# genometools/vstree

Hardware: AMD Instinct MI355X
Metric: queries/sec (100 bp queries, vmatch -mum -l 20 semantics, 3 Gbp ESA index resident in HBM) (higher is better)
Workload: dtype u8; 1 GPU; 3 Gbp synthetic DNA index, 10 M x 100 bp queries per GPU, -mum -l 20; index_bp=3000000000, queries_per_gpu=10000000, query_len=100, minlen=20, prefixlength=13, index_bytes_hbm=115012207262, reads_in_hbm=two bits per symbol, 32 bytes per read (vsa_pack_reads), parallelism=index replicated, queries sharded x1

## Files before the change

vstree_amd/csrc/esa_device.hpp:

```cpp
#pragma once

#include "vsa_internal.hpp"
#include <type_traits>

#define VSA_ISSPECIAL(c) ((c) >= (uint8_t) VSA_WILDCARD)

__device__ __forceinline__ uint64_t vsa_load8(const uint8_t *p)
{
  uint64_t v;
  __builtin_memcpy(&v, p, 8);
  return v;
}

struct vsa_u128
{
  uint64_t lo, hi;
};

__device__ __forceinline__ vsa_u128 vsa_load16(const void *p)
{
  vsa_u128 v;
  __builtin_memcpy(&v, p, 16);
  return v;
}
// ... 324 lines not shown
      uint32_t bits;
      __builtin_memcpy(&bits, ix.spec64 + (b >> 3), 4);
      bits >>= (uint32_t) (b & 7u);
      const uint64_t have = 25, want = blast - b + 1;
      const uint32_t mask = want >= have ? (1u << have) - 1u
                                         : (1u << want) - 1u;
      if ((bits & mask) != 0)
      {
        return false;
      }
      b += have;
    }
  }
  lcplen = l;
  return true;
}

struct PackedQuery
{
  uint64_t w[4];
  uint32_t valid;
};

__device__ __forceinline__ uint64_t vsa_pq_window(const PackedQuery &pq,
                                                  uint32_t at)
{
  const uint32_t i = at >> 5, sh = 2u * (at & 31u);
  const uint64_t a = i == 0 ? pq.w[0]
                            : (i == 1 ? pq.w[1]
                                      : (i == 2 ? pq.w[2]
                                                : (i == 3 ? pq.w[3] : 0))),
                 b = i == 0 ? pq.w[1]
                            : (i == 1 ? pq.w[2] : (i == 2 ? pq.w[3] : 0));
  return sh != 0 ? (a << sh) | (b >> (64 - sh)) : a;
}

template <int BLK>
__device__ __forceinline__ void vsa_pq_stage(const DevQueries &qs, uint64_t q0,
                                             uint32_t m, uint32_t *lds,
                                             PackedQuery &pq)
{
  const uint64_t nhere = q0 < qs.nq ? (qs.nq - q0 < (uint64_t) BLK
                                           ? qs.nq - q0
                                           : (uint64_t) BLK)
                                    : 0;
  const uint32_t bytes = (uint32_t) nhere * m;
  const uint8_t *src = qs.symbols + q0 * m;
  for (uint32_t i = threadIdx.x; 16 * i < bytes; i += BLK)
  {
    const vsa_u128 v = vsa_load16(src + 16 * (uint64_t) i);
    uint4 *dst = reinterpret_cast<uint4 *>(lds) + i;
    *dst = make_uint4((uint32_t) v.lo, (uint32_t) (v.lo >> 32),
                      (uint32_t) v.hi, (uint32_t) (v.hi >> 32));
  }
  __syncthreads();
  pq.w[0] = pq.w[1] = pq.w[2] = pq.w[3] = 0;
  pq.valid = 0;
  if (threadIdx.x < nhere)
  {
    const uint32_t *row = lds + threadIdx.x * (m >> 2);
    uint32_t firstbad = m;
#pragma unroll
    for (uint32_t j = 0; j < 32; j++)
    {
      if (4 * j < m)
      {
        const uint32_t x = row[j];
        const uint32_t bad = x & 0xFCFCFCFCu;
        if (bad != 0 && firstbad == m)
        {
          firstbad = 4 * j + ((uint32_t) __builtin_ctz(bad) >> 3);
        }
        pq.w[j >> 3] |= (uint64_t) (vsa_pack4top(x) >> 24)
                        << (56 - 8 * (j & 7));
      }
    }
    pq.valid = firstbad;
  }
}

__device__ __forceinline__ void vsa_pq_from_row(const DevQueries &qs,
                                                uint64_t q, uint32_t m,
                                                PackedQuery &pq, QSrc &src)
{
  const uint32_t W = qs.roww;
  const uint64_t *row = qs.rows + q * W;
  const vsa_u128 a = vsa_load16(row), b = vsa_load16(row + 2);
  const uint64_t last = W == 1 ? a.lo : (W == 2 ? a.hi : (W == 3 ? b.lo : b.hi));
  pq.w[0] = a.lo;
  pq.w[1] = W > 1 ? a.hi : 0;
  pq.w[2] = W > 2 ? b.lo : 0;
  pq.w[3] = W > 3 ? b.hi : 0;
  if (W == 1)
  {
    pq.w[0] &= ~0xFFull;
  } else if (W == 2)
  {
    pq.w[1] &= ~0xFFull;
  } else if (W == 3)
  {
    pq.w[2] &= ~0xFFull;
  } else
  {
    pq.w[3] &= ~0xFFull;
  }
  pq.valid = m;
  src.row = row;
  src.bytes = nullptr;
  src.pos = 0;
  src.m = (int32_t) m;
  if ((last & 0xFFu) != 0 && qs.nside > 0)
  {
    const uint64_t k = (a.lo >> 8) < qs.nside ? (a.lo >> 8) : qs.nside - 1;
    const uint8_t *sym = qs.side + k * (uint64_t) m;
    uint32_t firstbad = m;
    src.bytes = sym;
#pragma unroll
    for (int wi = 0; wi < 4; wi++)
    {
      uint64_t acc = 0;
      for (uint32_t k = 0; k < 32; k++)
      {
        const uint32_t j = 32u * (uint32_t) wi + k;
        if (j < m)
        {
          const uint8_t c = sym[j];
          if (c > 3 && firstbad == m)
          {
            firstbad = j;
          }
          acc |= (uint64_t) (c & 3u) << (62 - 2 * k);
        }
      }
      pq.w[wi] = acc;
    }
    pq.valid = firstbad;
  }
}

struct RowQuery
{
  const uint64_t *row;
  uint32_t valid;
};

__device__ __forceinline__ uint64_t vsa_pq_window(const RowQuery &rq,
                                                  uint32_t at)
{
  const uint32_t i = at >> 5, sh = 2u * (at & 31u);
  const vsa_u128 w = vsa_load16(rq.row + i);
  return sh != 0 ? (w.lo << sh) | (w.hi >> (64 - sh)) : w.lo;
}

__device__ __forceinline__ bool vsa_row_of(const DevQueries &qs, uint64_t q,
                                           uint32_t m, RowQuery &rq,
                                           QSrc &src)
{
  const uint32_t W = qs.roww;
  rq.row = qs.rows + q * W;
  rq.valid = m;
  src.row = rq.row;
  src.bytes = nullptr;
  src.pos = 0;
  src.m = (int32_t) m;
  const bool flagged = (rq.row[W - 1] & 0xFFu) != 0 && qs.nside > 0;
  if (flagged)
  {
    const uint64_t k0 = rq.row[0] >> 8,
                   k = k0 < qs.nside ? k0 : qs.nside - 1;
    src.bytes = qs.side + k * (uint64_t) m;
  }
  return flagged;
}

__device__ __forceinline__ uint8_t vsa_pq_symbol(const PackedQuery &pq,
                                                 uint32_t i)
{
  return (uint8_t) (vsa_pq_window(pq, i) >> 62);
}

template <int CHUNKS, typename IDX, typename QT>
__device__ __forceinline__ bool
vsa_extend_packed_pq(const DevIndex<IDX> &ix, uint64_t sufstart,
                     const QT &pq, uint32_t pqoff,
                     uint32_t querylen, uint32_t &lcplen)
{
  const uint32_t from = lcplen,
                 left = pq.valid > pqoff ? pq.valid - pqoff : 0;
  uint32_t l = lcplen, qeff = querylen < left ? querylen : left;
  bool open = true;

  if ((uint64_t) qeff > ix.n - sufstart)
  {
    qeff = (uint32_t) (ix.n - sufstart);
  }
  while (open && l < qeff)
  {
    uint64_t A[CHUNKS][2];
#pragma unroll
    for (int c = 0; c < CHUNKS; c++)
    {
      const uint32_t lc = l + 60u * (uint32_t) c;
      A[c][0] = A[c][1] = 0;
      if (c == 0 || lc < qeff)
      {
        const uint64_t pos = sufstart + lc;
        const uint32_t sh = 2u * (uint32_t) (pos & 3u);
        const vsa_u128 t = vsa_load16(ix.tis2 + (pos >> 2));
        const uint64_t t0 = __builtin_bswap64(t.lo),
                       t1 = __builtin_bswap64(t.hi);
        A[c][0] = sh != 0 ? (t0 << sh) | (t1 >> (64 - sh)) : t0;
        A[c][1] = t1 << sh;
      }
    }
#pragma unroll
    for (int c = 0; c < CHUNKS; c++)
    {
      if (open && l < qeff)
      {
        const uint64_t x0 = A[c][0] ^ vsa_pq_window(pq, pqoff + l),
                       x1 = (A[c][1] ^ vsa_pq_window(pq, pqoff + l + 32)) &
                            ~0xFFull;
        uint32_t same = 60;
        if (x0 != 0)
        {
          same = (uint32_t) __builtin_clzll(x0) >> 1;
        } else if (x1 != 0)
        {
          same = 32 + ((uint32_t) __builtin_clzll(x1) >> 1);
        }
        l += same;
        open = same == 60;
      }
    }
  }
  if (l > qeff)
  {
    l = qeff;
  }
  if (sufstart + l + 64 >= ix.firstspecial)
  {
    uint64_t b = (sufstart + from) >> 6;
    const uint64_t blast = (sufstart + l) >> 6;
    while (b <= blast)
    {
      uint32_t bits;
      __builtin_memcpy(&bits, ix.spec64 + (b >> 3), 4);
      bits >>= (uint32_t) (b & 7u);
      const uint64_t have = 25, want = blast - b + 1;
      const uint32_t mask = want >= have ? (1u << have) - 1u
                                         : (1u << want) - 1u;
      if ((bits & mask) != 0)
      {
        return false;
      }
      b += have;
    }
  }
  lcplen = l;
  return true;
}

template <typename IDX, bool KEYED>
__device__ __forceinline__ uint64_t vsa_sufstart(const DevIndex<IDX> &ix,
                                                 uint64_t i)
{
  return (KEYED && sizeof(IDX) == 4) ? (ix.esa8[i] & 0xFFFFFFFFull)
                                     : (uint64_t) ix.suf[i];
}

template <typename IDX>
__device__ __forceinline__ uint64_t vsa_entrystart(const DevIndex<IDX> &ix,
                                                   uint64_t entry, uint64_t w)
{
  if constexpr (sizeof(IDX) == 4)
  {
    return entry & 0xFFFFFFFFull;
  } else
  {
    return (uint64_t) ix.suf[w];
  }
}

#define VSA_WIDE_LEFTBITS 40
template <typename IDX>
__device__ __forceinline__ void vsa_slotbounds(uint64_t b, uint64_t &left,
                                               uint32_t &cnt)
{
  if constexpr (sizeof(IDX) == 4)
  {
    const uint32_t dl = (uint32_t) b, dm = (uint32_t) (b >> 32);
    left = dl;
    cnt = (dm > dl) ? dm - dl : 0;
  } else
  {
    left = b & ((1ull << VSA_WIDE_LEFTBITS) - 1);
    cnt = (uint32_t) (b >> VSA_WIDE_LEFTBITS);
  }
}

template <typename IDX, bool KEYED>
__device__ __forceinline__ uint32_t vsa_lcpbyte(const DevIndex<IDX> &ix,
                                                uint64_t i)
{
  return KEYED ? (uint32_t) (ix.esa8[i] >> 32) & 0xFFu : (uint32_t) ix.lcp[i];
}
// ... 89 lines not shown
    {
      return mid;
    }
  }
  return l;
}

template <typename IDX>
__device__ __forceinline__ uint64_t vsa_largelcp(const DevIndex<IDX> &ix,
                                                 uint64_t i)
{
  uint64_t lo = 0, hi = ix.nllv;

  while (lo < hi)
  {
    const uint64_t mid = lo + ((hi - lo) >> 1);
    const uint64_t k = (uint64_t) ix.llv[2 * mid];
    if (i < k)
    {
      hi = mid;
    } else if (i > k)
    {
      lo = mid + 1;
    } else
    {
      return (uint64_t) ix.llv[2 * mid + 1];
    }
  }
  return 255;
}

template <typename IDX>
__device__ __forceinline__ uint64_t vsa_evallcp(const DevIndex<IDX> &ix,
                                                uint64_t i)
{
  const uint64_t v = ix.lcp[i];
  return (v < 255) ? v : vsa_largelcp(ix, i);
}

template <typename IDX, typename QP = const uint8_t *>
__device__ __forceinline__ bool vsa_qgram2code(const DevIndex<IDX> &ix,
                                               QP qgram, uint64_t &code)
{
  uint64_t c = 0;
  bool ok = true;

  if (ix.numofchars == 4)
  {
    for (uint32_t i = 0; i < ix.pl; i++)
    {
      const uint8_t a = vsa_qsym(qgram, i);
      ok = ok && !VSA_ISSPECIAL(a);
      c = (c << 2) | (a & 3);
    }
  } else
  {
    for (uint32_t i = 0; i < ix.pl; i++)
    {
      const uint8_t a = vsa_qsym(qgram, i);
      ok = ok && !VSA_ISSPECIAL(a);
      c = c * ix.numofchars + a;
    }
  }
  code = c;
  return ok;
}

template <typename IDX, typename QP = const uint8_t *>
__device__ __forceinline__ bool vsa_bucket(const DevIndex<IDX> &ix, QP qgram,
                                           uint64_t &vleft, uint64_t &vright)
{
  uint64_t code;

  if (!vsa_qgram2code(ix, qgram, code))
  {
    return false;
  }
  vleft = (uint64_t) ix.bck[2 * code];
  vright = (uint64_t) ix.bck[2 * code + 1];
  if (vright <= vleft)
  {
    return false;
  }
  vright--;
  return true;
}

template <typename IDX, typename QP = const uint8_t *>
__device__ __forceinline__ bool
vsa_locate_reference(const DevIndex<IDX> &ix, QP query, uint32_t querylen,
                     uint32_t &maxlcp, uint64_t &witness)
{
  uint64_t vleft, vright;

  if (!vsa_bucket(ix, query, vleft, vright))
  {
    return false;
  }
  vsa_findmaxprefixlen(ix, vleft, vright, ix.pl, query, querylen, maxlcp,
                       witness);
  return true;
}


__device__ __forceinline__ uint64_t vsa_pack8(uint64_t w)
{
  uint64_t x = __builtin_bswap64(w) & 0x0303030303030303ull;
  x = (x | (x >> 6)) & 0x000F000F000F000Full;
  x = (x | (x >> 12)) & 0x000000FF000000FFull;
  x = (x | (x >> 24)) & 0xFFFFull;
  return x;
}

__device__ __forceinline__ uint32_t vsa_keylcp(uint32_t a, uint32_t b,
                                               uint32_t nsyms)
{
  const uint32_t x = (a ^ b) & ((1u << (2 * nsyms)) - 1u);
  if (x == 0)
  {
    return nsyms;
  }
  const uint32_t h = 31u - (uint32_t) __builtin_clz(x);
  return (2 * nsyms - 1 - h) >> 1;
}

enum
{
  VSA_LOC_NONE = 0,
  VSA_LOC_FOUND = 1,
  VSA_LOC_SLOW = 2
};

__device__ __forceinline__ uint64_t vsa_ld_entry(const uint64_t *p)
{
  return *p;
}

struct DeepHit
{
  uint64_t ew;
  uint32_t lcpnext;
  uint8_t leftsym;
  bool notleftmax;
};

struct DeepFront
{
  uint64_t left;
  uint64_t first;
  uint32_t cnt, qkey, limit;
  int state;
};

template <bool PQ = false, typename IDX = uint32_t, typename QT = PackedQuery,
          typename QP = const uint8_t *>
__device__ __forceinline__ void
vsa_deep_front(const DevIndex<IDX> &ix, bool active, QP query,
               uint32_t querylen, DeepFront &f,
               const QT *pq = nullptr, uint32_t pqoff = 0)
{
  const uint32_t D = ix.D;
  f.state = VSA_LOC_NONE;
  f.left = 0;
  f.cnt = f.qkey = f.limit = 0;
  f.first = 0;
  if (active)
  {
    uint32_t valid = 32;
    uint64_t S = 0;
    if (PQ)
    {
      const uint32_t left = pq->valid > pqoff ? pq->valid - pqoff : 0;
      valid = left < 32 ? left : 32;
      S = vsa_pq_window(*pq, pqoff);
    } else
    {
      const vsa_u128 qlo = vsa_load16(query), qhi = vsa_load16(query + 16u);
      const uint64_t w0 = qlo.lo, w1 = qlo.hi, w2 = qhi.lo, w3 = qhi.hi;
      const uint64_t notdna = 0xFCFCFCFCFCFCFCFCull;
      const uint64_t s0 = w0 & notdna, s1 = w1 & notdna, s2 = w2 & notdna,
                     s3 = w3 & notdna;
      if ((s0 | s1 | s2 | s3) != 0)
      {
        if (s0 != 0)
        {
          valid = (uint32_t) __builtin_ctzll(s0) >> 3;
        } else if (s1 != 0)
        {
          valid = 8 + ((uint32_t) __builtin_ctzll(s1) >> 3);
        } else if (s2 != 0)
        {
          valid = 16 + ((uint32_t) __builtin_ctzll(s2) >> 3);
        } else
        {
          valid = 24 + ((uint32_t) __builtin_ctzll(s3) >> 3);
        }
      }
      S = ((uint64_t) vsa_pack16(w0, w1) << 32) | vsa_pack16(w2, w3);
    }
    if (valid > querylen)
    {
      valid = querylen;
    }
    if (valid < ix.pl)
    {
      f.state = VSA_LOC_NONE;
    } else if (valid < D)
    {
      f.state = VSA_LOC_SLOW;
    } else
    {
      const uint64_t code = S >> (64 - 2 * D);
      f.qkey = (uint32_t) (S >> (64 - 2 * D - 2 * VSA_KEYSYMS)) & VSA_KEYMASK;
      f.limit = valid - D;
      if (f.limit > VSA_KEYSYMS)
      {
        f.limit = VSA_KEYSYMS;
      }
      const vsa_u128 sl = vsa_load16(ix.slot16 + 2 * code);
      f.first = sl.hi;
      vsa_slotbounds<IDX>(sl.lo, f.left, f.cnt);
      f.state = (f.cnt > 0) ? VSA_LOC_FOUND : VSA_LOC_NONE;
    }
  }
}

template <int AHEAD, bool PQ, typename IDX, typename QT,
          typename QP = const uint8_t *>
__device__ __forceinline__ void
vsa_extend_tie(const DevIndex<IDX> &ix, uint64_t sstart, QP query,
               uint32_t querylen, uint32_t &maxlcp, const QT *pq,
               uint32_t pqoff)
{
  uint32_t lcplen = maxlcp;
  bool done = false;
  if (ix.tis2 != nullptr)
  {
    if constexpr (PQ)
    {
      done = vsa_extend_packed_pq<(AHEAD > 1 ? 2 : 1)>(ix, sstart, *pq, pqoff,
                                                       querylen, lcplen);
    } else
    {
      done = vsa_extend_packed<(AHEAD > 1 ? 2 : 1)>(ix, sstart, query,
                                                    querylen, lcplen);
    }
  }
  if (!done)
  {
    lcplen = maxlcp;
    (void) vsa_compare32<IDX, AHEAD>(ix, sstart, query, querylen, lcplen);
  }
  maxlcp = lcplen;
}

template <int AHEAD = 1, bool PQ = false, typename IDX = uint32_t,
          typename QT = PackedQuery, typename QP = const uint8_t *>
__device__ __forceinline__ int
vsa_locate_deep_from(const DevIndex<IDX> &ix, const DeepFront &f, QP query,
                     uint32_t querylen, uint32_t &maxlcp,
                     uint64_t &w, DeepHit &hit, uint32_t needleft = 0xFFFFFFFFu,
                     uint32_t qleft = 0x100u, const QT *pq = nullptr,
                     uint32_t pqoff = 0)
{
  const uint32_t D = ix.D;
  int state = f.state;
  const typename std::conditional<sizeof(IDX) == 4, uint32_t, uint64_t>::type
      dl = (typename std::conditional<sizeof(IDX) == 4, uint32_t,
                                      uint64_t>::type) f.left;
  const uint32_t cnt = f.cnt, qkey = f.qkey, limit = f.limit;
  const uint64_t first = f.first;

  const bool searching = state == VSA_LOC_FOUND;
  const uint32_t qk = qkey >> (2 * (VSA_KEYSYMS - limit));

  const bool small = searching && cnt <= 4;
  const uint32_t ksh = 2 * (VSA_KEYSYMS - limit);
  uint64_t e[5] = {0, 0, 0, 0, 0};
  if (small && cnt == 1)
  {
    e[0] = first;
  } else if (small)
  {
    const uint64_t *p = ix.esa8 + (uint64_t) dl + 1;
    const vsa_u128 e12 = vsa_load16(p);
    e[0] = first;
    e[1] = e12.lo;
    e[2] = e12.hi;
    if (cnt > 2)
    {
      const vsa_u128 e34 = vsa_load16(p + 2);
      e[3] = e34.lo;
      e[4] = e34.hi;
    }
  }
  uint32_t lo = 0;
  bool flagged = false;
  bool anylong = false, allnotleft = true;
  const uint32_t enough = needleft < D + limit ? needleft : D + limit;
  if (small)
  {
#pragma unroll
    for (uint32_t i = 0; i < 4; i++)
    {
      if (i < cnt)
      {
        flagged = flagged || (e[i] & VSA_KEYFLAG) != 0;
        const uint32_t tk =
            ((uint32_t) (e[i] >> VSA_KEYSHIFT) & VSA_KEYMASK) >> ksh;
        lo += (tk < qk) ? 1u : 0u;
        if (qleft < 0x100u)
        {
          const bool islong = D + vsa_keylcp(tk, qk, limit) >= enough;
          const bool sameleft =
              (e[i] & VSA_LEFTSPECIAL) == 0 &&
              (uint32_t) ((e[i] >> VSA_LEFTSHIFT) & 3u) == qleft;
          anylong = anylong || islong;
          allnotleft = allnotleft && (!islong || sameleft);
        }
      }
    }
  }
  uint32_t hi = (searching && !small) ? cnt : 0;
  uint32_t maxcnt = hi;
  if (__ballot(hi != 0) != 0)
  {
#pragma unroll
    for (int d = 32; d >= 1; d >>= 1)
    {
      const uint32_t o = __shfl_xor(maxcnt, d, 64);
      maxcnt = o > maxcnt ? o : maxcnt;
    }
  }
  for (uint32_t span = maxcnt; span > 0; span >>= 1)
  {
    if (lo < hi)
    {
      const uint32_t mid = (lo + hi) >> 1;
      const uint64_t em = vsa_ld_entry(ix.esa8 + (uint64_t) dl + mid);
      flagged = flagged || (em & VSA_KEYFLAG) != 0;
      const uint32_t tk =
          ((uint32_t) (em >> VSA_KEYSHIFT) & VSA_KEYMASK) >> ksh;
      if (tk < qk)
      {
        lo = mid + 1;
      } else
      {
        hi = mid;
      }
    }
  }
  uint64_t epred = 0, esucc = 0, enext = 0;
  bool haspred = false, hassucc = false, hasnext = false;
  if (searching)
  {
    haspred = lo > 0;
    hassucc = lo < cnt;
    hasnext = lo + 1 < cnt;
    if (small)
    {
      epred = lo == 1 ? e[0] : (lo == 2 ? e[1] : (lo == 3 ? e[2] : e[3]));
      esucc = lo == 0 ? e[0]
                      : (lo == 1 ? e[1]
                                 : (lo == 2 ? e[2] : (lo == 3 ? e[3] : e[4])));
      enext = lo == 0 ? e[1] : (lo == 1 ? e[2] : (lo == 2 ? e[3] : e[4]));
    } else
    {
      const uint64_t base = (uint64_t) dl + lo;
      if (base > 0)
      {
        epred = vsa_ld_entry(ix.esa8 + base - 1);
      }
      if (base <= ix.n)
      {
        esucc = vsa_ld_entry(ix.esa8 + base);
      }
      if (base + 1 <= ix.n)
// ... 229 lines not shown
```

vstree_amd/csrc/mum_walk.inc:

```
template <typename IDX, bool DEEP, bool PQ, typename QP>
__device__ __forceinline__ void
vsa_walk_step(const DevIndex<IDX> &ix, const DevQueries &qs, bool &active,
              QP read, const RowQuery *rq, uint32_t qlen, uint32_t first,
              uint32_t &off, uint64_t q, const uint64_t *__restrict__ base,
              uint32_t perquery, uint32_t searchlength,
              vsa_match *__restrict__ out, uint64_t *__restrict__ outkey,
              uint64_t shardcap, uint32_t shard,
              unsigned long long *__restrict__ cursors, uint32_t packbits,
              uint32_t valbits, uint32_t &locates)
{
  uint32_t c = 0, maxlcp = 0;
  uint64_t witness = 0;
  uint8_t leftchar = (uint8_t) VSA_SEPARATOR;
  const uint32_t remaining = qlen - off;
  const QP qptr = read + off;
  bool have = false, fast = false;
  DeepHit hit;
  int st = VSA_LOC_SLOW;
  locates += active ? 1u : 0u;
  if (active && off > 0)
  {
    if constexpr (PQ)
    {
      leftchar = (uint8_t) (vsa_pq_window(*rq, off - 1) >> 62);
    } else
    {
      leftchar = vsa_qsym(read, off - 1);
    }
  }
  if constexpr (DEEP)
  {
    const uint32_t qleft = off > 0 ? (uint32_t) leftchar : 0x100u;
    if constexpr (PQ)
    {
      st = vsa_locate_deep<1, true>(ix, active, qptr, remaining, maxlcp,
                                    witness, hit, searchlength, qleft, rq,
                                    off);
    } else
    {
      st = vsa_locate_deep(ix, active, qptr, remaining, maxlcp, witness,
                           hit, searchlength, qleft);
    }
  }
  if (st == VSA_LOC_SLOW)
  {
    have = active &&
           vsa_locate_reference(ix, qptr, remaining, maxlcp, witness);
  } else
  {
    have = st == VSA_LOC_FOUND;
    fast = have && maxlcp < 255;
  }
  const bool cutshort = st != VSA_LOC_SLOW && hit.notleftmax;
  if (have && maxlcp >= searchlength && !cutshort)
  {
    if (fast)
    {
      const uint32_t lcpw = (uint32_t) (hit.ew >> 32) & 0xFFu;
      const bool unique = (witness == 0 || lcpw < maxlcp) &&
                          (witness + 1 > ix.n - 1 || hit.lcpnext < maxlcp);
      c = (unique && (VSA_ISSPECIAL(leftchar) || leftchar != hit.leftsym))
              ? 1u
              : 0u;
    } else
    {
      c = (vsa_mum_candidate<IDX, DEEP>(ix, maxlcp, witness) &&
           vsa_leftmaximal(ix, vsa_sufstart<IDX, DEEP>(ix, witness),
                           leftchar))
              ? 1u
              : 0u;
    }
  }
  const uint64_t inshard = vsa_wave_reserve01(
      cursors + (uint64_t) shard * VSA_CURSOR_STRIDE, c != 0);
  if (c != 0 && inshard < shardcap)
  {
    const uint64_t dbstart = fast ? vsa_entrystart(ix, hit.ew, witness)
                                  : vsa_sufstart<IDX, DEEP>(ix, witness);
    const uint64_t t0 = (base != nullptr) ? base[q] : q * perquery;
    vsa_write_candidate(qs, out, outkey,
                        (uint64_t) shard * shardcap + inshard, q, off,
                        t0 + off, dbstart, maxlcp, packbits, valbits);
  }
  if (active)
  {
    uint32_t bound;
    if (st == VSA_LOC_SLOW)
    {
      bound = have ? maxlcp : ix.pl - 1;
    } else
    {
      bound = have ? maxlcp : ix.D - 1;
    }
    const uint32_t reach = off + bound;
    uint32_t next = off - 1;
    bool left = off > first;
    if (!cutshort && reach + 1 < off + searchlength)
    {
      left = left && reach >= searchlength;
      next = reach - searchlength;
    }
    active = left && next >= first;
    off = next;
  }
}

template <typename IDX, bool DEEP, bool PQ, typename QP>
__device__ __forceinline__ uint32_t
vsa_walk_chunk(const DevIndex<IDX> &ix, const DevQueries &qs, bool active,
               QP read, const RowQuery *rq, uint32_t qlen, uint32_t first,
               uint32_t off, uint64_t q, const uint64_t *__restrict__ base,
               uint32_t perquery, uint32_t searchlength,
               vsa_match *__restrict__ out, uint64_t *__restrict__ outkey,
               uint64_t shardcap, uint32_t shard,
               unsigned long long *__restrict__ cursors, uint32_t packbits,
               uint32_t valbits)
{
  uint32_t locates = 0;
  while (__any(active))
  {
    vsa_walk_step<IDX, DEEP, PQ>(ix, qs, active, read, rq, qlen, first, off, q,
                                 base, perquery, searchlength, out, outkey,
                                 shardcap, shard, cursors, packbits, valbits,
                                 locates);
  }
  return locates;
}
```

vstree_amd/csrc/mum_workplan.inc:

```



#define VSA_PLAN_RANGES 4
#define VSA_PLAN_ROUNDS 6
#define VSA_PLAN_UNKNOWN 0xFFFFFFFFu

#ifndef VSA_PLAN_WAVES
#define VSA_PLAN_WAVES 1
#endif
#ifndef VSA_FIRST_WAVES
#define VSA_FIRST_WAVES 1
#endif
struct PlanRanges
{
  uint32_t r[VSA_PLAN_RANGES];
};

__device__ __forceinline__ void plan_add(PlanRanges &pr, uint32_t &nr,
                                         uint32_t first, uint32_t last)
{
  if (first > last)
  {
    return;
  }
// ... 389 lines not shown
      rel[0] = 0;
    }
    __syncthreads();
    for (uint32_t d = 1; d < BLK; d <<= 1)
    {
      const uint64_t v = (tid + 1 > d) ? lanesum[tid + 1 - d] : 0;
      __syncthreads();
      lanesum[tid + 1] += v;
      __syncthreads();
    }
#pragma unroll
    for (int k = 0; k < RPT; k++)
    {
      rel[tid * RPT + k + 1] = (uint32_t) lanesum[tid] + mine[k];
    }
    __syncthreads();
  }
  const uint32_t total = rel[RPB];
  if (tid == 0)
  {
    if constexpr (MUM)
    {
      blocksum[vsa_bid()].offsets = lanesum[BLK] >> 32;
    } else
    {
      blocksum[vsa_bid()] = PlannedWork{total, total};
    }
  }
  const uint32_t shard = vsa_bid() & shardmask;
  uint32_t locates = 0;
  for (uint32_t i0 = 0; i0 < total; i0 += BLK)
  {
    const uint32_t i = i0 + tid;
    bool active = i < total;
    uint32_t off = 0, first = 0, qlen = qs.uniformlen;
    uint64_t q = 0, t0 = 0;
    const uint8_t *qstart = qs.symbols;
    if (active)
    {
      uint32_t lo = 0, hi = RPB;
      while (hi - lo > 1)
      {
        const uint32_t mid = (lo + hi) >> 1;
        if (rel[mid] <= i)
        {
          lo = mid;
        } else
        {
          hi = mid;
        }
      }
      uint32_t r = i - rel[lo];
#pragma unroll
      for (int k = 0; k < VSA_PLAN_RANGES; k++)
      {
        const uint32_t rf = pr[lo].r[k] & 0xFFFFu, len = pr[lo].r[k] >> 16,
                       nchunks = (len + chunk - 1) >> cshift;
        if (r < nchunks)
        {
          const uint32_t at = r << cshift,
                         n = len - at < chunk ? len - at : chunk;
          first = rf + at;
          off = first + n - 1;
          r = 0xFFFFFFFFu;
        } else if (r != 0xFFFFFFFFu)
        {
          r -= nchunks;
        }
      }
      q = q0 + lo;
      if constexpr (!MUM)
      {
        t0 = (base != nullptr) ? base[q] : q * perquery;
      }
      if constexpr (MUM && !ROWS)
      {
        if (qs.dense)
        {
          qstart = qs.symbols + q * qs.uniformlen;
        } else
        {
          qstart = qs.symbols + qs.start[q];
          qlen = (uint32_t) qs.length[q];
        }
      }
    }
    if constexpr (!MUM)
    {
      vsa_query_item<IDX, false, DEEP>(ix, qs, active, q, off, t0 + off,
                                       searchlength, out, outkey, shardcap,
                                       shard, cursors, 0, 0);
      continue;
    }
    if constexpr (DEEP && ROWS)
    {
      RowQuery rq;
      QSrc src;
      bool flagged = false;
      rq.row = qs.rows;
      rq.valid = 0;
      src.row = qs.rows;
      src.bytes = nullptr;
      src.pos = src.m = 0;
      if (active)
      {
        flagged = vsa_row_of(qs, q, qs.uniformlen, rq, src);
      }
      locates += vsa_walk_chunk<IDX, true, true>(
          ix, qs, active && !flagged, src, &rq, qlen, first, off, q, base,
          perquery, searchlength, out, outkey, shardcap, shard, cursors,
          packbits, valbits);
      if (__any(active && flagged))
      {
        locates += vsa_walk_chunk<IDX, true, false>(
            ix, qs, active && flagged, src, nullptr, qlen, first, off, q, base,
            perquery, searchlength, out, outkey, shardcap, shard, cursors,
            packbits, valbits);
      }
    } else
    {
      locates += vsa_walk_chunk<IDX, DEEP, false>(
          ix, qs, active, qstart, nullptr, qlen, first, off, q, base, perquery,
          searchlength, out, outkey, shardcap, shard, cursors, packbits,
          valbits);
    }
  }
  if constexpr (MUM)
  {
#pragma unroll
    for (int d = 32; d >= 1; d >>= 1)
    {
      locates += __shfl_xor(locates, d, 64);
    }
    if ((tid & 63u) == 0)
    {
      wavelocates[tid >> 6] = locates;
    }
    __syncthreads();
    if (tid == 0)
    {
      uint32_t s = 0;
#pragma unroll
      for (int w = 0; w < BLK / 64; w++)
      {
        s += wavelocates[w];
      }
      blocksum[vsa_bid()].locates = s;
    }
  }
}

struct WalkTile
{
  PlanRanges pr[64];
  uint32_t q[64];
  uint32_t pre[65];
};
#define VSA_WALK_ASIDE 128
struct WalkAside
{
  uint32_t q[VSA_WALK_ASIDE], r[VSA_WALK_ASIDE];
};

__device__ __forceinline__ void vsa_wave_lds_fence()
{
  __builtin_amdgcn_fence(__ATOMIC_RELEASE, "wavefront");
  __builtin_amdgcn_wave_barrier();
  __builtin_amdgcn_fence(__ATOMIC_ACQUIRE, "wavefront");
}

__device__ __forceinline__ uint32_t vsa_rank_in(uint64_t mask)
{
  return __builtin_amdgcn_mbcnt_hi(
      (uint32_t) (mask >> 32), __builtin_amdgcn_mbcnt_lo((uint32_t) mask, 0u));
}

__device__ __forceinline__ void vsa_plan_chunk(const PlanRanges &p, uint32_t r,
                                               uint32_t cshift,
                                               uint32_t &first, uint32_t &off)
{
  const uint32_t chunk = 1u << cshift;
#pragma unroll
  for (int k = 0; k < VSA_PLAN_RANGES; k++)
  {
    const uint32_t rf = p.r[k] & 0xFFFFu, len = p.r[k] >> 16,
                   nchunks = (len + chunk - 1) >> cshift;
    if (r < nchunks)
    {
      const uint32_t at = r << cshift, n = len - at < chunk ? len - at : chunk;
      first = rf + at;
      off = first + n - 1;
      r = 0xFFFFFFFFu;
    } else if (r != 0xFFFFFFFFu)
    {
      r -= nchunks;
    }
  }
}

template <typename IDX, bool DEEP = true, bool ROWS = false>
__global__ void __launch_bounds__(256, VSA_WALK_WAVES)
k_mum_walk_tiles(const DevIndex<IDX> ix, const DevQueries qs,
                 const uint64_t *__restrict__ base, uint32_t perquery,
                 const PlanRanges *__restrict__ plan,
                 const uint32_t *__restrict__ plancount,
                 const uint32_t *__restrict__ list,
                 const uint64_t *__restrict__ nlistword,
                 unsigned long long *__restrict__ tilecounter,
                 uint32_t searchlength, vsa_match *__restrict__ out,
                 uint64_t *__restrict__ outkey, uint64_t shardcap,
                 uint32_t shardmask, unsigned long long *__restrict__ cursors,
                 uint32_t packbits, uint32_t valbits,
                 PlannedWork *__restrict__ blocksum, uint32_t chunkshift)
{
  __shared__ WalkTile tiles[4];
  __shared__ WalkAside asides[ROWS ? 4 : 1];
  const uint32_t lane = threadIdx.x & 63u, wave = threadIdx.x >> 6;
  WalkTile &tile = tiles[wave];
  WalkAside &aside = asides[ROWS ? wave : 0];
  const uint64_t nlist = *nlistword & 0xFFFFFFFFull;
  const uint32_t shard = vsa_bid() & shardmask;
  uint32_t head = 0, tail = 0, naside = 0;
  bool exhausted = false;
  bool active = false;
  uint32_t off = 0, first = 0, q = 0, qlen = qs.uniformlen;
  uint32_t locates = 0, offsets = 0;
  const uint8_t *qstart = qs.symbols;
  for (;;)
  {
    uint64_t freemask = __ballot(!active);
    while (freemask != 0 && !(ROWS && naside >= 64))
    {
      if (head == tail)
      {
        if (exhausted)
        {
          break;
        }
        unsigned long long mine = 0;
        if (lane == 0)
        {
          mine = atomicAdd(tilecounter, 1ull);
        }
        const uint64_t t0 =
            ((uint64_t) __builtin_amdgcn_readfirstlane((uint32_t) (mine >> 32))
             << 32) |
            __builtin_amdgcn_readfirstlane((uint32_t) mine);
        if (t0 * 64 >= nlist)
        {
          exhausted = true;
          break;
        }
        const uint64_t t = t0 * 64 + lane;
        uint32_t tq = 0, nch = 0;
        PlanRanges p;
#pragma unroll
        for (int g = 0; g < VSA_PLAN_RANGES; g++)
        {
          p.r[g] = 0;
        }
        if (t < nlist)
        {
          tq = list[t];
          const uint32_t c = plancount[tq];
          p = plan[tq];
          offsets += c;
          if (c > 0)
          {
#pragma unroll
            for (int g = 0; g < VSA_PLAN_RANGES; g++)
            {
              nch += ((p.r[g] >> 16) + (1u << chunkshift) - 1) >> chunkshift;
            }
          }
        }
        const uint32_t incl = vsa_wave_inclusive_sum(nch);
        vsa_wave_lds_fence();
        tile.q[lane] = tq;
        tile.pr[lane] = p;
        tile.pre[lane + 1] = incl;
        if (lane == 0)
        {
          tile.pre[0] = 0;
        }
        vsa_wave_lds_fence();
        head = 0;
        tail = __builtin_amdgcn_readlane(incl, 63);
        continue;
      }
      const uint32_t nfree = (uint32_t) __popcll(freemask),
                     take = nfree < tail - head ? nfree : tail - head,
                     rank = vsa_rank_in(freemask);
      const bool took = !active && rank < take;
      bool flagged = false;
      if (took)
      {
        const uint32_t i = head + rank;
        uint32_t lo = 0;
#pragma unroll
        for (uint32_t d = 32; d >= 1; d >>= 1)
        {
          if (tile.pre[lo + d] <= i)
          {
            lo += d;
          }
        }
        q = tile.q[lo];
        vsa_plan_chunk(tile.pr[lo], i - tile.pre[lo], chunkshift, first, off);
        if constexpr (ROWS)
        {
          RowQuery rq;
          QSrc src;
          flagged = vsa_row_of(qs, q, qs.uniformlen, rq, src);
        } else
        {
          if (qs.dense)
          {
            qstart = qs.symbols + (uint64_t) q * qs.uniformlen;
          } else
          {
            qstart = qs.symbols + qs.start[q];
            qlen = (uint32_t) qs.length[q];
          }
        }
        active = !flagged;
      }
      head += take;
      if constexpr (ROWS)
      {
        const uint64_t fmask = __ballot(flagged);
        if (flagged)
        {
          const uint32_t at = naside + vsa_rank_in(fmask);
          aside.q[at] = q;
          aside.r[at] = first | (off << 16);
        }
        naside += (uint32_t) __popcll(fmask);
      }
      freemask = __ballot(!active);
    }
    if (!__any(active))
    {
      if constexpr (ROWS)
      {
        if (naside > 0)
        {
          vsa_wave_lds_fence();
          for (uint32_t a0 = 0; a0 < naside; a0 += 64)
          {
            const bool mine = a0 + lane < naside;
            uint32_t aq = 0, afirst = 0, aoff = 0;
            RowQuery arq;
            QSrc src;
            arq.row = qs.rows;
            arq.valid = 0;
            src.row = qs.rows;
            src.bytes = nullptr;
            src.pos = src.m = 0;
            if (mine)
            {
              aq = aside.q[a0 + lane];
              afirst = aside.r[a0 + lane] & 0xFFFFu;
              aoff = aside.r[a0 + lane] >> 16;
              (void) vsa_row_of(qs, aq, qs.uniformlen, arq, src);
            }
            locates += vsa_walk_chunk<IDX, true, false>(
                ix, qs, mine, src, nullptr, qlen, afirst, aoff, aq, base,
                perquery, searchlength, out, outkey, shardcap, shard, cursors,
                packbits, valbits);
          }
          vsa_wave_lds_fence();
          naside = 0;
          q = first = off = 0;
          continue;
        }
      }
      break;
    }
    if constexpr (DEEP && ROWS)
    {
      RowQuery rq;
      QSrc src;
      rq.row = qs.rows + (uint64_t) q * qs.roww;
      rq.valid = qlen;
      src.row = rq.row;
      src.bytes = nullptr;
      src.pos = 0;
      src.m = (int32_t) qlen;
      vsa_walk_step<IDX, true, true>(ix, qs, active, src, &rq, qlen, first,
                                     off, q, base, perquery, searchlength, out,
                                     outkey, shardcap, shard, cursors, packbits,
                                     valbits, locates);
    } else
    {
      vsa_walk_step<IDX, DEEP, false>(ix, qs, active, qstart, nullptr, qlen,
                                      first, off, q, base, perquery,
                                      searchlength, out, outkey, shardcap,
                                      shard, cursors, packbits, valbits,
                                      locates);
    }
  }
  uint64_t sum = locates | ((uint64_t) offsets << 32);
#pragma unroll
  for (int d = 32; d >= 1; d >>= 1)
  {
    sum += vsa_shfl64(sum, (int) lane ^ d);
  }
  if (lane == 0)
  {
    blocksum[vsa_bid() * 4 + wave] =
        PlannedWork{sum & 0xFFFFFFFFull, sum >> 32};
  }
}

template <typename IDX, bool DEEP, bool PQ = false, bool ROWS = false,
          bool WINDOWS = false>
__global__ void __launch_bounds__(VSA_BLOCK, VSA_FIRST_WAVES)
k_mum_first(const DevIndex<IDX> ix, const DevQueries qs, uint32_t perquery,
            uint32_t searchlength, uint32_t *__restrict__ count,
            uint32_t *__restrict__ firste, uint32_t *__restrict__ fmlen,
            uint64_t *__restrict__ fmdb,
            uint64_t *__restrict__ blockcount = nullptr)
{
  extern __shared__ uint32_t stagedqueries[];
  __shared__ uint32_t wantwaves[VSA_BLOCK / 64], candwaves[VSA_BLOCK / 64];
  const uint64_t q = vsa_bid() * VSA_BLOCK + threadIdx.x;
  uint32_t qlen = qs.uniformlen, perq = perquery;
  const uint8_t *qptr = qs.symbols;
  uint32_t maxlcp = 0;
  uint64_t witness = 0;
  bool have = false, fast = false;
  DeepHit hit;

  if (!ROWS && q < qs.nq)
  {
    if (qs.dense)
    {
      qptr = qs.symbols + q * qs.uniformlen;
    } else
    {
      qptr = qs.symbols + qs.start[q];
      qlen = (uint32_t) qs.length[q];
      perq = (qlen >= searchlength) ? qlen - searchlength + 1 : 0;
    }
  }
  const bool active = q < qs.nq && perq > 0;
  if constexpr (DEEP && ROWS && WINDOWS)
  {
    RowQuery rq;
    QSrc src;
    bool flagged = false;
    rq.row = qs.rows;
    rq.valid = 0;
    src.row = qs.rows;
    src.bytes = nullptr;
    src.pos = src.m = 0;
    if (q < qs.nq)
    {
      flagged = vsa_row_of(qs, q, qlen, rq, src);
    }
    int st = vsa_locate_deep<3, true>(ix, active && !flagged, src, qlen,
                                      maxlcp, witness, hit, 0xFFFFFFFFu,
                                      0x100u, &rq, 0);
    if (active && flagged)
    {
      st = VSA_LOC_SLOW;
    }
    if (st == VSA_LOC_SLOW)
    {
      have = vsa_locate_reference(ix, src, qlen, maxlcp, witness);
    } else
    {
      have = st == VSA_LOC_FOUND;
      fast = have && maxlcp < 255;
    }
  } else if constexpr (DEEP && ROWS)
  {
    PackedQuery pq;
    QSrc src;
    pq.w[0] = pq.w[1] = pq.w[2] = pq.w[3] = 0;
    pq.valid = 0;
    src.row = qs.rows;
    src.bytes = nullptr;
    src.pos = src.m = 0;
    if (q < qs.nq)
    {
      vsa_pq_from_row(qs, q, qlen, pq, src);
    }
    const int st = vsa_locate_deep<3, true>(ix, active, src, qlen, maxlcp,
                                            witness, hit, 0xFFFFFFFFu, 0x100u,
                                            &pq);
    if (st == VSA_LOC_SLOW)
    {
      have = vsa_locate_reference(ix, src, qlen, maxlcp, witness);
    } else
    {
      have = st == VSA_LOC_FOUND;
      fast = have && maxlcp < 255;
    }
  } else if constexpr (DEEP)
  {
    int st;
    if constexpr (PQ)
    {
      PackedQuery pq;
      vsa_pq_stage<VSA_BLOCK>(qs, vsa_bid() * VSA_BLOCK, qlen,
                              stagedqueries, pq);
      st = vsa_locate_deep<3, true>(ix, active, qptr, qlen, maxlcp,
                                           witness, hit, 0xFFFFFFFFu, 0x100u,
                                           &pq);
    } else
    {
      st = vsa_locate_deep<3>(ix, active, qptr, qlen, maxlcp, witness, hit);
    }
    if (st == VSA_LOC_SLOW)
    {
      have = vsa_locate_reference(ix, qptr, qlen, maxlcp, witness);
    } else
    {
      have = st == VSA_LOC_FOUND;
      fast = have && maxlcp < 255;
    }
  } else
  {
    if (active)
    {
      have = vsa_locate_reference(ix, qptr, qlen, maxlcp, witness);
    }
  }
  uint32_t len = 0, wanted = 0;
  if (q < qs.nq)
  {
    uint64_t db = 0;
    if (active && have && maxlcp >= searchlength)
    {
      bool unique;
      if (fast)
      {
        const uint32_t lcpw = (uint32_t) (hit.ew >> 32) & 0xFFu;
        unique = (witness == 0 || lcpw < maxlcp) &&
                 (witness + 1 > ix.n - 1 || hit.lcpnext < maxlcp);
        db = vsa_entrystart(ix, hit.ew, witness);
      } else
      {
        unique = vsa_mum_candidate<IDX, DEEP>(ix, maxlcp, witness);
        db = vsa_sufstart<IDX, DEEP>(ix, witness);
      }
      len = unique ? maxlcp : 0;
    }
    wanted = !active ? 0 : ((have && maxlcp >= qlen) ? 0 : perq);
    fmlen[q] = len;
    fmdb[q] = db;
    firste[q] = (active && have) ? maxlcp : VSA_PLAN_UNKNOWN;
    count[q] = wanted;
  }
  if (blockcount != nullptr)
  {
    const uint64_t wmask = __ballot(wanted > 0), cmask = __ballot(len != 0);
    if ((threadIdx.x & 63) == 0)
    {
      wantwaves[threadIdx.x >> 6] = (uint32_t) __popcll(wmask);
      candwaves[threadIdx.x >> 6] = (uint32_t) __popcll(cmask);
    }
    __syncthreads();
// ... 115 lines not shown
```

Measured before the change: 4.181 billion queries/s.

## Prefetch work tiles, precompute flag masks, and keep walk counters wave-uniform

Each wave's first tile is now assigned statically, and the atomic fetch for the next tile is issued right after staging the current one. This hides the atomic latency. Each query's side-table flag is read once at tile load and turned into a ballot mask, so the per-chunk row read is gone. The locate and offset counters become scalar via readfirstlane, which removes the final shuffle reduction. The packed-row walk step also fetches the left character and the 32-symbol window with a single 16-byte load, and the tile ranges are stored as uint4 for vectorized LDS access. The risks are in tile-counter semantics, which now need the counter offset by the wave count, and in the correctness of the new window shift logic.

```diff
diff --git a/vstree_amd/csrc/esa_device.hpp b/vstree_amd/csrc/esa_device.hpp
--- a/vstree_amd/csrc/esa_device.hpp
+++ b/vstree_amd/csrc/esa_device.hpp
@@ -500,6 +500,21 @@
   return sh != 0 ? (w.lo << sh) | (w.hi >> (64 - sh)) : w.lo;
 }
 
+__device__ __forceinline__ uint64_t vsa_row_step_window(const RowQuery &rq,
+                                                        uint32_t off,
+                                                        uint8_t &leftchar)
+{
+  const uint32_t at = off > 0 ? off - 1 : 0;
+  const vsa_u128 w = vsa_load16(rq.row + (at >> 5));
+  const uint32_t s = off > 0 ? (at & 31u) + 1 : 0;
+  if (off > 0)
+  {
+    leftchar = (uint8_t) ((w.lo >> (64 - 2 * s)) & 3u);
+  }
+  return s == 0 ? w.lo
+                : (s == 32 ? w.hi : (w.lo << (2 * s)) | (w.hi >> (64 - 2 * s)));
+}
+
 __device__ __forceinline__ bool vsa_row_of(const DevQueries &qs, uint64_t q,
                                            uint32_t m, RowQuery &rq,
                                            QSrc &src)
@@ -895,6 +910,45 @@
   int state;
 };
 
+template <typename IDX>
+__device__ __forceinline__ void
+vsa_deep_front_window(const DevIndex<IDX> &ix, bool active, uint64_t S,
+                      uint32_t valid, uint32_t querylen, DeepFront &f)
+{
+  const uint32_t D = ix.D;
+  f.state = VSA_LOC_NONE;
+  f.left = 0;
+  f.cnt = f.qkey = f.limit = 0;
+  f.first = 0;
+  if (active)
+  {
+    if (valid > querylen)
+    {
+      valid = querylen;
+    }
+    if (valid < ix.pl)
+    {
+      f.state = VSA_LOC_NONE;
+    } else if (valid < D)
+    {
+      f.state = VSA_LOC_SLOW;
+    } else
+    {
+      const uint64_t code = S >> (64 - 2 * D);
+      f.qkey = (uint32_t) (S >> (64 - 2 * D - 2 * VSA_KEYSYMS)) & VSA_KEYMASK;
+      f.limit = valid - D;
+      if (f.limit > VSA_KEYSYMS)
+      {
+        f.limit = VSA_KEYSYMS;
+      }
+      const vsa_u128 sl = vsa_load16(ix.slot16 + 2 * code);
+      f.first = sl.hi;
+      vsa_slotbounds<IDX>(sl.lo, f.left, f.cnt);
+      f.state = (f.cnt > 0) ? VSA_LOC_FOUND : VSA_LOC_NONE;
+    }
+  }
+}
+
 template <bool PQ = false, typename IDX = uint32_t, typename QT = PackedQuery,
           typename QP = const uint8_t *>
 __device__ __forceinline__ void
@@ -902,15 +956,10 @@
                uint32_t querylen, DeepFront &f,
                const QT *pq = nullptr, uint32_t pqoff = 0)
 {
-  const uint32_t D = ix.D;
-  f.state = VSA_LOC_NONE;
-  f.left = 0;
-  f.cnt = f.qkey = f.limit = 0;
-  f.first = 0;
+  uint32_t valid = 32;
+  uint64_t S = 0;
   if (active)
   {
-    uint32_t valid = 32;
-    uint64_t S = 0;
     if (PQ)
     {
       const uint32_t left = pq->valid > pqoff ? pq->valid - pqoff : 0;
@@ -941,31 +990,8 @@
       }
       S = ((uint64_t) vsa_pack16(w0, w1) << 32) | vsa_pack16(w2, w3);
     }
-    if (valid > querylen)
-    {
-      valid = querylen;
-    }
-    if (valid < ix.pl)
-    {
-      f.state = VSA_LOC_NONE;
-    } else if (valid < D)
-    {
-      f.state = VSA_LOC_SLOW;
-    } else
-    {
-      const uint64_t code = S >> (64 - 2 * D);
-      f.qkey = (uint32_t) (S >> (64 - 2 * D - 2 * VSA_KEYSYMS)) & VSA_KEYMASK;
-      f.limit = valid - D;
-      if (f.limit > VSA_KEYSYMS)
-      {
-        f.limit = VSA_KEYSYMS;
-      }
-      const vsa_u128 sl = vsa_load16(ix.slot16 + 2 * code);
-      f.first = sl.hi;
-      vsa_slotbounds<IDX>(sl.lo, f.left, f.cnt);
-      f.state = (f.cnt > 0) ? VSA_LOC_FOUND : VSA_LOC_NONE;
-    }
-  }
+  }
+  vsa_deep_front_window(ix, active, S, valid, querylen, f);
 }
 
 template <int AHEAD, bool PQ, typename IDX, typename QT,
diff --git a/vstree_amd/csrc/mum_walk.inc b/vstree_amd/csrc/mum_walk.inc
--- a/vstree_amd/csrc/mum_walk.inc
+++ b/vstree_amd/csrc/mum_walk.inc
@@ -18,12 +18,16 @@
   DeepHit hit;
   int st = VSA_LOC_SLOW;
   locates += active ? 1u : 0u;
-  if (active && off > 0)
+  uint64_t window = 0;
+  if constexpr (PQ)
   {
-    if constexpr (PQ)
+    if (active)
     {
-      leftchar = (uint8_t) (vsa_pq_window(*rq, off - 1) >> 62);
-    } else
+      window = vsa_row_step_window(*rq, off, leftchar);
+    }
+  } else
+  {
+    if (active && off > 0)
     {
       leftchar = vsa_qsym(read, off - 1);
     }
@@ -33,9 +37,13 @@
     const uint32_t qleft = off > 0 ? (uint32_t) leftchar : 0x100u;
     if constexpr (PQ)
     {
-      st = vsa_locate_deep<1, true>(ix, active, qptr, remaining, maxlcp,
-                                    witness, hit, searchlength, qleft, rq,
-                                    off);
+      const uint32_t left = rq->valid > off ? rq->valid - off : 0;
+      DeepFront f;
+      vsa_deep_front_window(ix, active, window, left < 32 ? left : 32,
+                            remaining, f);
+      st = vsa_locate_deep_from<1, true>(ix, f, qptr, remaining, maxlcp,
+                                         witness, hit, searchlength, qleft,
+                                         rq, off);
     } else
     {
       st = vsa_locate_deep(ix, active, qptr, remaining, maxlcp, witness,
diff --git a/vstree_amd/csrc/mum_workplan.inc b/vstree_amd/csrc/mum_workplan.inc
--- a/vstree_amd/csrc/mum_workplan.inc
+++ b/vstree_amd/csrc/mum_workplan.inc
@@ -565,7 +565,7 @@
 
 struct WalkTile
 {
-  PlanRanges pr[64];
+  alignas(16) PlanRanges pr[64];
   uint32_t q[64];
   uint32_t pre[65];
 };
@@ -586,6 +586,15 @@
 {
   return __builtin_amdgcn_mbcnt_hi(
       (uint32_t) (mask >> 32), __builtin_amdgcn_mbcnt_lo((uint32_t) mask, 0u));
+}
+
+__device__ __forceinline__ uint32_t vsa_lane_here()
+{
+  uint32_t l;
+  asm volatile("v_mbcnt_lo_u32_b32 %0, -1, 0\n\t"
+               "v_mbcnt_hi_u32_b32 %0, -1, %0"
+               : "=v"(l));
+  return l;
 }
 
 __device__ __forceinline__ void vsa_plan_chunk(const PlanRanges &p, uint32_t r,
@@ -628,13 +637,16 @@
 {
   __shared__ WalkTile tiles[4];
   __shared__ WalkAside asides[ROWS ? 4 : 1];
-  const uint32_t lane = threadIdx.x & 63u, wave = threadIdx.x >> 6;
+  const uint32_t wave = __builtin_amdgcn_readfirstlane(threadIdx.x >> 6);
   WalkTile &tile = tiles[wave];
   WalkAside &aside = asides[ROWS ? wave : 0];
   const uint64_t nlist = *nlistword & 0xFFFFFFFFull;
   const uint32_t shard = vsa_bid() & shardmask;
   uint32_t head = 0, tail = 0, naside = 0;
   bool exhausted = false;
+  uint64_t flagmask = 0;
+  const uint32_t nwaves = (uint32_t) vsa_nblocks() * 4u;
+  uint32_t nexttile = (uint32_t) vsa_bid() * 4u + wave;
   bool active = false;
   uint32_t off = 0, first = 0, q = 0, qlen = qs.uniformlen;
   uint32_t locates = 0, offsets = 0;
@@ -650,22 +662,16 @@
         {
           break;
         }
-        unsigned long long mine = 0;
-        if (lane == 0)
-        {
-          mine = atomicAdd(tilecounter, 1ull);
-        }
-        const uint64_t t0 =
-            ((uint64_t) __builtin_amdgcn_readfirstlane((uint32_t) (mine >> 32))
-             << 32) |
-            __builtin_amdgcn_readfirstlane((uint32_t) mine);
+        const uint64_t t0 = __builtin_amdgcn_readfirstlane(nexttile);
         if (t0 * 64 >= nlist)
         {
           exhausted = true;
           break;
         }
+        const uint32_t lane = vsa_lane_here();
         const uint64_t t = t0 * 64 + lane;
-        uint32_t tq = 0, nch = 0;
+        uint32_t tq = 0, nch = 0, planned = 0;
+        bool special = false;
         PlanRanges p;
 #pragma unroll
         for (int g = 0; g < VSA_PLAN_RANGES; g++)
@@ -677,7 +683,13 @@
           tq = list[t];
           const uint32_t c = plancount[tq];
           p = plan[tq];
-          offsets += c;
+          if constexpr (ROWS)
+          {
+            special = qs.nside > 0 &&
+                      (qs.rows[(uint64_t) tq * qs.roww + qs.roww - 1] &
+                       0xFFu) != 0;
+          }
+          planned = c;
           if (c > 0)
           {
 #pragma unroll
@@ -688,9 +700,13 @@
           }
         }
         const uint32_t incl = vsa_wave_inclusive_sum(nch);
+        offsets = __builtin_amdgcn_readfirstlane(
+            offsets +
+            __builtin_amdgcn_readlane(vsa_wave_inclusive_sum(planned), 63));
         vsa_wave_lds_fence();
         tile.q[lane] = tq;
-        tile.pr[lane] = p;
+        *reinterpret_cast<uint4 *>(&tile.pr[lane]) =
+            make_uint4(p.r[0], p.r[1], p.r[2], p.r[3]);
         tile.pre[lane + 1] = incl;
         if (lane == 0)
         {
@@ -699,6 +715,14 @@
         vsa_wave_lds_fence();
         head = 0;
         tail = __builtin_amdgcn_readlane(incl, 63);
+        if constexpr (ROWS)
+        {
+          flagmask = __ballot(special);
+        }
+        if (lane == 0)
+        {
+          nexttile = nwaves + atomicAdd((unsigned int *) tilecounter, 1u);
+        }
         continue;
       }
       const uint32_t nfree = (uint32_t) __popcll(freemask),
@@ -719,12 +743,13 @@
           }
         }
         q = tile.q[lo];
-        vsa_plan_chunk(tile.pr[lo], i - tile.pre[lo], chunkshift, first, off);
+        const uint32_t before = tile.pre[lo];
+        const uint4 ranges = *reinterpret_cast<const uint4 *>(&tile.pr[lo]);
+        vsa_plan_chunk(PlanRanges{{ranges.x, ranges.y, ranges.z, ranges.w}},
+                       i - before, chunkshift, first, off);
         if constexpr (ROWS)
         {
-          RowQuery rq;
-          QSrc src;
-          flagged = vsa_row_of(qs, q, qs.uniformlen, rq, src);
+          flagged = ((flagmask >> lo) & 1u) != 0;
         } else
         {
           if (qs.dense)
@@ -759,6 +784,7 @@
         if (naside > 0)
         {
           vsa_wave_lds_fence();
+          const uint32_t lane = vsa_lane_here();
           for (uint32_t a0 = 0; a0 < naside; a0 += 64)
           {
             const bool mine = a0 + lane < naside;
@@ -777,10 +803,14 @@
               aoff = aside.r[a0 + lane] >> 16;
               (void) vsa_row_of(qs, aq, qs.uniformlen, arq, src);
             }
-            locates += vsa_walk_chunk<IDX, true, false>(
-                ix, qs, mine, src, nullptr, qlen, afirst, aoff, aq, base,
-                perquery, searchlength, out, outkey, shardcap, shard, cursors,
-                packbits, valbits);
+            locates = __builtin_amdgcn_readfirstlane(
+                locates +
+                __builtin_amdgcn_readlane(
+                    vsa_wave_inclusive_sum(vsa_walk_chunk<IDX, true, false>(
+                        ix, qs, mine, src, nullptr, qlen, afirst, aoff, aq,
+                        base, perquery, searchlength, out, outkey, shardcap,
+                        shard, cursors, packbits, valbits)),
+                    63));
           }
           vsa_wave_lds_fence();
           naside = 0;
@@ -790,6 +820,9 @@
       }
       break;
     }
+    locates = __builtin_amdgcn_readfirstlane(
+        locates + (uint32_t) __popcll(__ballot(active)));
+    uint32_t counted = 0;
     if constexpr (DEEP && ROWS)
     {
       RowQuery rq;
@@ -803,26 +836,19 @@
       vsa_walk_step<IDX, true, true>(ix, qs, active, src, &rq, qlen, first,
                                      off, q, base, perquery, searchlength, out,
                                      outkey, shardcap, shard, cursors, packbits,
-                                     valbits, locates);
+                                     valbits, counted);
     } else
     {
       vsa_walk_step<IDX, DEEP, false>(ix, qs, active, qstart, nullptr, qlen,
                                       first, off, q, base, perquery,
                                       searchlength, out, outkey, shardcap,
                                       shard, cursors, packbits, valbits,
-                                      locates);
-    }
-  }
-  uint64_t sum = locates | ((uint64_t) offsets << 32);
-#pragma unroll
-  for (int d = 32; d >= 1; d >>= 1)
-  {
-    sum += vsa_shfl64(sum, (int) lane ^ d);
-  }
-  if (lane == 0)
-  {
-    blocksum[vsa_bid() * 4 + wave] =
-        PlannedWork{sum & 0xFFFFFFFFull, sum >> 32};
+                                      counted);
+    }
+  }
+  if (vsa_lane_here() == 0)
+  {
+    blocksum[vsa_bid() * 4 + wave] = PlannedWork{locates, offsets};
   }
 }
 
```

New measurement: 4.261 billion queries/s (median of 6 runs). Within noise of the previous version (+1.9%).
